# GuyTevet/motion-diffusion-model

Measured on NVIDIA H100. Metric: motions/sec, higher is better.
Workload: dtype fp16 operands / fp32 accumulate (in/out projections hi-lo split)

## Files before the change

motion-diffusion-model_b200/csrc/attention_tc.cuh:

```cuda
#pragma once
#include <cuda_fp16.h>

#include "epilogues.cuh"
#include "ptx.cuh"

namespace b200 {

constexpr int ATC_THREADS = 256;
constexpr int ATC_QROWS = 128;
constexpr int ATC_DH = 128;
constexpr int ATC_MAX_KEYS = 256;

struct AttnTcSmem {
  static __host__ __device__ int total(int keys) { return 1024 + 4 * keys * 128; }
};

template <bool WIDE>
__global__ void __launch_bounds__(ATC_THREADS, 2)
attention_tc_kernel(const __grid_constant__ CUtensorMap map_kv, const __half* __restrict__ qkv, __half* __restrict__ out,
                    const int* __restrict__ kvlen, int S, int d, int keys, float scale_log2) {
  extern __shared__ uint8_t smem_raw[];
  __shared__ uint64_t bar_k, bar_v;
  const int atom = keys * 128;
  uint8_t* sK = reinterpret_cast<uint8_t*>((reinterpret_cast<uintptr_t>(smem_raw) + 1023) & ~uintptr_t(1023));
  uint8_t* sV = sK + 2 * atom;
  const int warp = threadIdx.x >> 5, lane = threadIdx.x & 31;
  const int h = blockIdx.x, smp = blockIdx.y, tile = blockIdx.z;
  const int ld = 3 * d;
  const __half* base = qkv + static_cast<size_t>(smp) * S * ld;

  pdl_launch_dependents();
  if (threadIdx.x == 0) {
    tma_prefetch_desc(&map_kv);
    mbar_init(&bar_k, 1);
    mbar_init(&bar_v, 1);
    fence_barrier_init();
  }
  __syncthreads();
  pdl_wait();
  if (threadIdx.x == 0) {
    mbar_expect_tx(&bar_k, 2 * atom);
    for (int a = 0; a < 2; ++a) tma_load_3d(sK + a * atom, &map_kv, &bar_k, d + h * ATC_DH + 64 * a, 0, smp);
    mbar_expect_tx(&bar_v, 2 * atom);
    for (int a = 0; a < 2; ++a) tma_load_3d(sV + a * atom, &map_kv, &bar_v, 2 * d + h * ATC_DH + 64 * a, 0, smp);
  }

  const int q0 = tile * ATC_QROWS + warp * 16;
  if (q0 >= S) return;
  const int g = lane >> 2, t = lane & 3;
  const int ra = q0 + g, rb = q0 + g + 8;
  const bool va = ra < S, vb = rb < S;
  uint32_t qa[8][4];
  {
    const uint32_t* pa = reinterpret_cast<const uint32_t*>(base + static_cast<size_t>(va ? ra : 0) * ld + h * ATC_DH);
    const uint32_t* pb = reinterpret_cast<const uint32_t*>(base + static_cast<size_t>(vb ? rb : 0) * ld + h * ATC_DH);
#pragma unroll
    for (int ks = 0; ks < 8; ++ks) {
      qa[ks][0] = va ? pa[8 * ks + t] : 0u;
      qa[ks][1] = vb ? pb[8 * ks + t] : 0u;
      qa[ks][2] = va ? pa[8 * ks + 4 + t] : 0u;
      qa[ks][3] = vb ? pb[8 * ks + 4 + t] : 0u;
    }
  }
  const int kvl = min(kvlen[smp], S);
  const int nblk = max(1, (kvl + 15) >> 4);
  const uint32_t r7 = lane & 7;
  const uint32_t k_row = smem_u32(sK) + ((lane & 7) + 8 * (lane >> 4)) * 128, k_hi = (lane >> 3) & 1;
  const uint32_t v_row = smem_u32(sV) + ((lane & 7) + 8 * ((lane >> 3) & 1)) * 128, v_hi = lane >> 4;
  auto swz = [&](uint32_t row_addr, uint32_t chunk) {
    return row_addr + (chunk >> 3) * atom + (((chunk & 7) ^ r7) << 4);
  };
  auto scores = [&](int kk, float (&s)[2][4]) {
#pragma unroll
    for (int n = 0; n < 2; ++n)
#pragma unroll
      for (int i = 0; i < 4; ++i) s[n][i] = 0.f;
#pragma unroll
    for (int ks = 0; ks < 8; ++ks) {
      uint32_t b[4];
      ldmatrix_x4(b, swz(k_row + 16 * kk * 128, 2 * ks + k_hi));
      mma_16816(s[0], qa[ks], b[0], b[1]);
      mma_16816(s[1], qa[ks], b[2], b[3]);
    }
  };
  mbar_wait(&bar_k, 0);
  float mxa = -INFINITY, mxb = -INFINITY;
#pragma unroll 1
  for (int kk = 0; kk < nblk; ++kk) {
    float s[2][4];
    scores(kk, s);
#pragma unroll
    for (int n = 0; n < 2; ++n)
#pragma unroll
      for (int i = 0; i < 2; ++i) {
        const int key = 16 * kk + 8 * n + 2 * t + i;
        if (key < kvl) {
          mxa = fmaxf(mxa, s[n][i]);
          mxb = fmaxf(mxb, s[n][2 + i]);
        }
      }
  }
#pragma unroll
  for (int o = 1; o < 4; o <<= 1) {
    mxa = fmaxf(mxa, __shfl_xor_sync(0xffffffffu, mxa, o));
    mxb = fmaxf(mxb, __shfl_xor_sync(0xffffffffu, mxb, o));
  }
  const float offa = (mxa == -INFINITY) ? 0.f : mxa * scale_log2;
  const float offb = (mxb == -INFINITY) ? 0.f : mxb * scale_log2;
  auto ex2 = [](float x) {
    float y;
    asm("ex2.approx.ftz.f32 %0, %1;" : "=f"(y) : "f"(x));
    return y;
  };
  float o[16][4];
#pragma unroll
  for (int j = 0; j < 16; ++j)
#pragma unroll
    for (int i = 0; i < 4; ++i) o[j][i] = 0.f;
  float suma = 0.f, sumb = 0.f;
  mbar_wait(&bar_v, 0);
#pragma unroll 1
  for (int kk = 0; kk < nblk; ++kk) {
    float s[2][4];
    scores(kk, s);
    uint32_t pa[4];
#pragma unroll
    for (int n = 0; n < 2; ++n) {
      const int key = 16 * kk + 8 * n + 2 * t;
      const float p0 = key < kvl ? ex2(fmaf(s[n][0], scale_log2, -offa)) : 0.f;
      const float p1 = key + 1 < kvl ? ex2(fmaf(s[n][1], scale_log2, -offa)) : 0.f;
      const float p2 = key < kvl ? ex2(fmaf(s[n][2], scale_log2, -offb)) : 0.f;
      const float p3 = key + 1 < kvl ? ex2(fmaf(s[n][3], scale_log2, -offb)) : 0.f;
      suma += p0 + p1;
      sumb += p2 + p3;
      pa[2 * n] = pack_half2(p0, p1);
      pa[2 * n + 1] = pack_half2(p2, p3);
    }
#pragma unroll
    for (int nd = 0; nd < 8; ++nd) {
      uint32_t b[4];
      ldmatrix_x4_trans(b, swz(v_row + 16 * kk * 128, 2 * nd + v_hi));
      mma_16816(o[2 * nd], pa, b[0], b[1]);
      mma_16816(o[2 * nd + 1], pa, b[2], b[3]);
    }
  }
#pragma unroll
  for (int off = 1; off < 4; off <<= 1) {
    suma += __shfl_xor_sync(0xffffffffu, suma, off);
    sumb += __shfl_xor_sync(0xffffffffu, sumb, off);
  }
  const float inva = suma > 0.f ? 1.f / suma : 0.f;
  const float invb = sumb > 0.f ? 1.f / sumb : 0.f;
  const int ldo = (WIDE ? 2 : 1) * d;
  __half* oa = out + (static_cast<size_t>(smp) * S + (va ? ra : 0)) * ldo + h * ATC_DH + 2 * t;
  __half* ob = out + (static_cast<size_t>(smp) * S + (vb ? rb : 0)) * ldo + h * ATC_DH + 2 * t;
#pragma unroll
  for (int j = 0; j < 16; ++j) {
    const float x0 = o[j][0] * inva, x1 = o[j][1] * inva, x2 = o[j][2] * invb, x3 = o[j][3] * invb;
    const __half2 ha = __floats2half2_rn(x0, x1), hb = __floats2half2_rn(x2, x3);
    if (va) *reinterpret_cast<__half2*>(oa + 8 * j) = ha;
    if (vb) *reinterpret_cast<__half2*>(ob + 8 * j) = hb;
    if (WIDE) {
      const float2 fa = __half22float2(ha), fb = __half22float2(hb);
      if (va) *reinterpret_cast<__half2*>(oa + d + 8 * j) = __floats2half2_rn(x0 - fa.x, x1 - fa.y);
      if (vb) *reinterpret_cast<__half2*>(ob + d + 8 * j) = __floats2half2_rn(x2 - fb.x, x3 - fb.y);
    }
  }
}

}
```

motion-diffusion-model_b200/csrc/engine.cu:

```cuda
#include <cuda.h>
#include <cuda_fp16.h>
#include <cuda_runtime.h>

#include <cmath>
#include <cstdarg>
#include <cstdio>
#include <cstring>
#include <map>
#include <string>
#include <vector>

#include "../../include/b200mdm.h"
#include "attention_tc.cuh"
#include "epilogues.cuh"
#include "gemm.cuh"
#include "gemm_ln.cuh"
#include "postprocess.cuh"
#include "kernels.cuh"

using namespace b200;

static thread_local char g_err[512] = "";
static int fail(int code, const char* fmt, ...) {
  va_list ap;
// ... 166 lines not shown
  if (zero) CUDA_TRY(cudaMemset(*p, 0, n * sizeof(T)));
  return B200MDM_OK;
}
template <class T>
static void dfree(T*& p) {
  if (p) cudaFree(p);
  p = nullptr;
}

template <int BN, class Epi, bool RES = false>
static int set_gemm_attr() {
  CUDA_TRY(cudaFuncSetAttribute(gemm_f16_wgmma<BN, Epi, RES>, cudaFuncAttributeMaxDynamicSharedMemorySize,
                                GemmSmem<BN, Epi, RES>::TOTAL));
  return B200MDM_OK;
}
static int init_kernel_attrs() {
  static unsigned long long done_mask = 0;
  int dev = 0;
  CUDA_TRY(cudaGetDevice(&dev));
  if (dev < 64 && ((done_mask >> dev) & 1ull)) return B200MDM_OK;
  TRY((set_gemm_attr<128, EpiBiasF16<false>>()));
  TRY((set_gemm_attr<128, EpiBiasF16<true>>()));
  TRY((set_gemm_attr<256, EpiBiasF16<false>>()));
  TRY((set_gemm_attr<256, EpiBiasF16<true>>()));
  TRY((set_gemm_attr<64, EpiBiasF16<false>, true>()));
  TRY((set_gemm_attr<64, EpiBiasF16<true>, true>()));
  TRY((set_gemm_attr<128, EpiBiasF16Wide<true>>()));
  TRY((set_gemm_attr<128, EpiBiasF16Global>()));
  CUDA_TRY(cudaFuncSetAttribute(gemm_resid_ln_cluster, cudaFuncAttributeMaxDynamicSharedMemorySize, GemmLnSmem::TOTAL));
  TRY((set_gemm_attr<128, EpiEmbed>()));
  TRY((set_gemm_attr<96, EpiOutStep>()));
  CUDA_TRY(cudaFuncSetAttribute(attention_tc_kernel<false>, cudaFuncAttributeMaxDynamicSharedMemorySize,
                                AttnTcSmem::total(ATC_MAX_KEYS)));
  CUDA_TRY(cudaFuncSetAttribute(attention_tc_kernel<true>, cudaFuncAttributeMaxDynamicSharedMemorySize,
                                AttnTcSmem::total(ATC_MAX_KEYS)));
  if (dev < 64) done_mask |= 1ull << dev;
  return B200MDM_OK;
}

static bool g_pdl_now = false;
static bool pdl_enabled() {
  static int v = -1;
  if (v < 0) {
    const char* e = getenv("B200MDM_PDL");
    v = (e && e[0] == '0') ? 0 : 1;
  }
  return v == 1;
}
struct PdlScope {
  PdlScope() { g_pdl_now = pdl_enabled(); }
// ... 44 lines not shown
                            const float* bias, cudaStream_t s, int num_sms) {
  typename EpiBiasF16<GELU>::Params p{bias};
  return launch_gemm<128, EpiBiasF16<GELU>>(a, b, c, M, N, K, p, s, num_sms);
}

static int launch_gemm_resid_ln(const CUtensorMap& a, const CUtensorMap& w256, const CUtensorMap& hres, int M, int K,
                                const float* bias, const float* gamma, const float* beta, cudaStream_t s, int num_sms) {
  const int tiles = (M + GEMM_BLOCK_M - 1) / GEMM_BLOCK_M;
  const int max_clusters = num_sms / 2;
  const int clusters = tiles < max_clusters ? tiles : max_clusters;
  GemmLnParams lp{bias, gamma, beta, 1e-5f};
  CUDA_TRY(launch_k(gemm_resid_ln_cluster, dim3(2 * clusters), dim3(GLN_THREADS), GemmLnSmem::TOTAL, s, a, w256, hres, M, K, lp));
  return B200MDM_OK;
}

static int launch_attention_tc(const CUtensorMap& map_kv, const __half* qkv, __half* out, const int* kvlen, int n_samples,
                               int S, int d, int H, cudaStream_t s, bool wide = false) {
  if (d != H * ATC_DH) return fail(B200MDM_ENOTIMPL, "attention: head_dim must be 128");
  if (S > ATC_MAX_KEYS) return fail(B200MDM_ENOTIMPL, "attention: at most %d tokens per sample", ATC_MAX_KEYS);
  const int keys = (S + 15) & ~15;
  const float scale_log2 = 1.4426950408889634f / sqrtf(static_cast<float>(ATC_DH));
  const dim3 grid(H, n_samples, (S + ATC_QROWS - 1) / ATC_QROWS);
  CUDA_TRY(launch_k(wide ? attention_tc_kernel<true> : attention_tc_kernel<false>, grid, dim3(ATC_THREADS), AttnTcSmem::total(keys),
                    s, map_kv, qkv, out, kvlen, S, d, keys, scale_log2));
  return B200MDM_OK;
}
#ifdef B200_TRACE
static int debug_skip_mask() {
  static int v = -1;
  if (v < 0) {
    const char* e = getenv("B200MDM_DEBUG_SKIP");
    v = e ? atoi(e) : 0;
  }
  return v;
}
#define B200_SKIP(bit) (debug_skip_mask() & (bit))
#else
#define B200_SKIP(bit) (0)
#endif
// ... 299 lines not shown
  if (e->dec) {
    TRY(dalloc(&e->qc16, M * d));
    TRY(make_map_t(&e->m_qc_st, e->qc16, 2, M, d, d, 32));
    e->Mt = 0;
    e->prefix_set = false;
  }
  e->B = B; e->T = T; e->S = S; e->halves = halves; e->Bp = Bp;
  e->M = static_cast<int>(M); e->MB = static_cast<int>(MB);
  attach_l2_window(e);
  TRY(make_map(&e->m_xin, e->xin16, MB, 3 * e->Kp_in, 3 * e->Kp_in, GEMM_BLOCK_M));
  TRY(make_map(&e->m_h16, e->hres, M, kw * d, 2 * d, GEMM_BLOCK_M));
  TRY(make_map(&e->m_att, e->att16, M, kw * d, kw * d, GEMM_BLOCK_M));
  TRY(make_map(&e->m_ffn, e->ffn16, M, kw * e->ff, kw * e->ff, GEMM_BLOCK_M));
  TRY(make_map(&e->m_g16, e->g16, static_cast<size_t>(B) * T, 3 * d, 3 * d, GEMM_BLOCK_M));
  TRY(make_map_t(&e->m_qkv_st, e->qkv16, 2, M, 3 * d, 3 * d, 32));
  TRY(make_map_3d(&e->m_qkv_kv, e->qkv16, Bp, S, 3 * d, 3 * d, (S + 15) & ~15));
  TRY(make_map_t(&e->m_ffn_st, e->ffn16, 2, M, kw * e->ff, kw * e->ff, 32));
  TRY(make_map_res(&e->m_res_c, e->hres, MB, d));
  TRY(make_map_res(&e->m_res_u, e->hres + (halves == 2 ? MB * d * 2 : 0), MB, d));
  TRY(make_hres_map(&e->m_hres, e->hres, M));
  TRY(dalloc(&e->pe_bias, static_cast<size_t>(S) * d));
  pe_bias_kernel<<<S, 128, 0, s>>>(e->pe_bias, e->pe, e->b_in, S, d);
  CUDA_TRY(cudaGetLastError());
  TRY(dalloc(&e->eps_buf, static_cast<size_t>(B) * e->JF * T));
  return B200MDM_OK;
}

static void attach_l2_window(b200mdm_engine* e, cudaStream_t stream) {
  cudaDeviceProp prop;
  int dev = 0;
  if (cudaGetDevice(&dev) == cudaSuccess && cudaGetDeviceProperties(&prop, dev) == cudaSuccess && prop.persistingL2CacheMaxSize > 0) {
// ... 632 lines not shown
  p.noise_batch_stride = (flags & B200MDM_FLAG_CONST_NOISE) ? 0 : static_cast<long long>(JF) * T;
  p.B = B; p.S = T; p.T = T; p.J = JF; p.mode = mode;
  p.s_off = 0;
  p.clip_denoised = (flags & B200MDM_FLAG_CLIP_DENOISED) ? 1 : 0;
  return launch_gemm<96, EpiOutStep>(m_g16, m_wout, m_g16, B * T, N_out_pad, 3 * d, p, s, sms);
}

extern "C" int b200mdm_test_attention(const void* qkv16_dev, void* out16_dev, const int32_t* kvlen_dev,
                                      int32_t n_samples, int32_t S, int32_t d, int32_t impl, void* stream) {
  if (!qkv16_dev || !out16_dev || !kvlen_dev || n_samples <= 0 || S <= 0) return fail(B200MDM_EINVAL, "bad argument");
  TRY(init_kernel_attrs());
  cudaStream_t s = static_cast<cudaStream_t>(stream);
  if (impl != 0 && impl != 1) return fail(B200MDM_EINVAL, "impl must be 0 (fp16 output) or 1 ([hi | lo] output)");
  if (S > ATC_MAX_KEYS) return fail(B200MDM_EINVAL, "attention handles at most %d tokens", ATC_MAX_KEYS);
  CUtensorMap mkv;
  TRY(make_map_3d(&mkv, qkv16_dev, n_samples, S, 3 * d, 3 * d, (S + 15) & ~15));
  return launch_attention_tc(mkv, static_cast<const __half*>(qkv16_dev), static_cast<__half*>(out16_dev), kvlen_dev, n_samples,
                             S, d, d / ATC_DH, s, impl == 1);
}

extern "C" int b200mdm_test_cross_attention(const void* q16_dev, const void* kv16_dev, const unsigned char* mask_dev,
                                            void* out16_dev, int32_t n_samples, int32_t S, int32_t n_tokens, int32_t ld_kv,
                                            void* stream) {
  const int d = 512;
  if (!q16_dev || !kv16_dev || !mask_dev || !out16_dev || n_samples <= 0 || S <= 0 || n_tokens <= 0 || n_tokens > 64 ||
      ld_kv < 2 * d || ld_kv % 8)
    return fail(B200MDM_EINVAL, "bad argument");
  cudaStream_t s = static_cast<cudaStream_t>(stream);
  const float sl2 = 1.4426950408889634f / sqrtf(128.0f);
  const dim3 cg(d / 128, n_samples), cb(128);
  const __half* q = static_cast<const __half*>(q16_dev);
// ... 12 lines not shown
      ld < 512 || ld % 8)
    return fail(B200MDM_EINVAL, "bad argument");
  TRY(init_kernel_attrs());
  int dev = 0, sms = 132;
  CUDA_TRY(cudaGetDevice(&dev));
  CUDA_TRY(cudaDeviceGetAttribute(&sms, cudaDevAttrMultiProcessorCount, dev));
  cudaStream_t s = static_cast<cudaStream_t>(stream);
  const int M = n_samples * S;
  __half* qkv = nullptr;
  CUDA_TRY(cudaMallocAsync(reinterpret_cast<void**>(&qkv), static_cast<size_t>(M) * 1536 * sizeof(__half), s));
  CUtensorMap ma, mb, mc, mkv;
  int r = make_map(&ma, h16_dev, M, 512, ld, GEMM_BLOCK_M);
  if (r == B200MDM_OK) r = make_map(&mb, wqkv16_dev, 1536, 512, 512, 128);
  if (r == B200MDM_OK) r = make_map_t(&mc, qkv, 2, M, 1536, 1536, 32);
  if (r == B200MDM_OK) r = launch_gemm_bias<false>(ma, mb, mc, M, 1536, 512, bqkv_dev, s, sms);
  if (r == B200MDM_OK) r = make_map_3d(&mkv, qkv, n_samples, S, 1536, 1536, (S + 15) & ~15);
  if (r == B200MDM_OK)
    r = launch_attention_tc(mkv, qkv, static_cast<__half*>(out16_dev), kvlen_dev, n_samples, S, 512, 4, s);
  CUDA_TRY(cudaFreeAsync(qkv, s));
  return r;
}

extern "C" int b200mdm_test_gemm_resid_ln(const void* a16_dev, const void* w16_dev, const float* bias_dev,
                                          const float* gamma_dev, const float* beta_dev, void* hres16_dev, int32_t M,
                                          int32_t K, void* stream) {
  if (!a16_dev || !w16_dev || !bias_dev || !gamma_dev || !beta_dev || !hres16_dev || M <= 0 || K <= 0 || K % 8)
    return fail(B200MDM_EINVAL, "bad argument");
  TRY(init_kernel_attrs());
  int dev = 0, sms = 132;
  CUDA_TRY(cudaGetDevice(&dev));
  CUDA_TRY(cudaDeviceGetAttribute(&sms, cudaDevAttrMultiProcessorCount, dev));
// ... 25 lines not shown
```

motion-diffusion-model_b200/csrc/ptx.cuh:

```cuda
#pragma once
#include <cuda.h>
#include <cuda_fp16.h>
#include <cuda_runtime.h>
#include <stdint.h>

namespace b200 {

__device__ __forceinline__ uint32_t smem_u32(const void* p) {
  return static_cast<uint32_t>(__cvta_generic_to_shared(p));
}

__device__ __forceinline__ bool elect_one() {
  uint32_t pred = 0;
  asm volatile(
      "{\n\t.reg .pred P;\n\t"
      "elect.sync _|P, 0xffffffff;\n\t"
      "selp.u32 %0, 1, 0, P;\n\t}\n"
      : "=r"(pred));
  return pred != 0;
}

__device__ __forceinline__ void mbar_init(uint64_t* bar, uint32_t count) {
  asm volatile("mbarrier.init.shared::cta.b64 [%0], %1;" ::"r"(smem_u32(bar)), "r"(count) : "memory");
}
// ... 106 lines not shown
}
__device__ __forceinline__ void st_async_f32x2(uint32_t remote_addr, float a, float b, uint32_t remote_bar) {
  asm volatile("st.async.shared::cluster.mbarrier::complete_tx::bytes.v2.f32 [%0], {%1, %2}, [%3];"
               ::"r"(remote_addr), "f"(a), "f"(b), "r"(remote_bar)
               : "memory");
}

__device__ __forceinline__ uint64_t wgmma_desc_k_sw128(uint32_t smem_addr) {
  uint64_t d = 0;
  d |= static_cast<uint64_t>((smem_addr & 0x3FFFF) >> 4);
  d |= static_cast<uint64_t>(1) << 16;
  d |= static_cast<uint64_t>(1024 >> 4) << 32;
  d |= static_cast<uint64_t>(1) << 62;
  return d;
}
__device__ __forceinline__ void wgmma_fence() { asm volatile("wgmma.fence.sync.aligned;" ::: "memory"); }
__device__ __forceinline__ void wgmma_commit() { asm volatile("wgmma.commit_group.sync.aligned;" ::: "memory"); }
template <int N>
__device__ __forceinline__ void wgmma_wait() {
  asm volatile("wgmma.wait_group.sync.aligned %0;" ::"n"(N) : "memory");
}
template <int NR>
__device__ __forceinline__ void wgmma_fence_acc(float (&d)[NR]) {
#pragma unroll
  for (int i = 0; i < NR; ++i) asm volatile("" : "+f"(d[i])::"memory");
}

template <int N> struct Wgmma;
#include "wgmma_ops.inc"

__device__ __forceinline__ void mma_16816(float (&c)[4], const uint32_t (&a)[4], uint32_t b0, uint32_t b1) {
  asm volatile("mma.sync.aligned.m16n8k16.row.col.f32.f16.f16.f32 {%0,%1,%2,%3}, {%4,%5,%6,%7}, {%8,%9}, {%0,%1,%2,%3};\n"
               : "+f"(c[0]), "+f"(c[1]), "+f"(c[2]), "+f"(c[3])
               : "r"(a[0]), "r"(a[1]), "r"(a[2]), "r"(a[3]), "r"(b0), "r"(b1));
}
__device__ __forceinline__ void ldmatrix_x4(uint32_t (&r)[4], uint32_t smem_addr) {
  asm volatile("ldmatrix.sync.aligned.m8n8.x4.shared.b16 {%0,%1,%2,%3}, [%4];"
               : "=r"(r[0]), "=r"(r[1]), "=r"(r[2]), "=r"(r[3]) : "r"(smem_addr));
}
__device__ __forceinline__ void ldmatrix_x4_trans(uint32_t (&r)[4], uint32_t smem_addr) {
  asm volatile("ldmatrix.sync.aligned.m8n8.x4.trans.shared.b16 {%0,%1,%2,%3}, [%4];"
               : "=r"(r[0]), "=r"(r[1]), "=r"(r[2]), "=r"(r[3]) : "r"(smem_addr));
}
// ... 3 lines not shown
```

motion-diffusion-model_b200/csrc/wgmma_ops.inc:

```
template <> struct Wgmma<64> {
  static constexpr int NREG = 32;
  static __device__ __forceinline__ void mma(float (&d)[32], uint64_t da, uint64_t db, uint32_t accumulate) {
    asm volatile(
        "{\n\t.reg .pred p;\n\tsetp.ne.b32 p, %34, 0;\n\t"
        "wgmma.mma_async.sync.aligned.m64n64k16.f32.f16.f16 {%0, %1, %2, %3, %4, %5, %6, %7, %8, %9, %10, %11, %12, %13, %14, %15, %16, %17, %18, %19, %20, %21, %22, %23, %24, %25, %26, %27, %28, %29, %30, %31}, %32, %33, p, 1, 1, 0, 0;\n\t}\n"
        : "+f"(d[0]), "+f"(d[1]), "+f"(d[2]), "+f"(d[3]), "+f"(d[4]), "+f"(d[5]), "+f"(d[6]), "+f"(d[7]), "+f"(d[8]), "+f"(d[9]), "+f"(d[10]), "+f"(d[11]), "+f"(d[12]), "+f"(d[13]), "+f"(d[14]), "+f"(d[15]), "+f"(d[16]), "+f"(d[17]), "+f"(d[18]), "+f"(d[19]), "+f"(d[20]), "+f"(d[21]), "+f"(d[22]), "+f"(d[23]), "+f"(d[24]), "+f"(d[25]), "+f"(d[26]), "+f"(d[27]), "+f"(d[28]), "+f"(d[29]), "+f"(d[30]), "+f"(d[31])
        : "l"(da), "l"(db), "r"(accumulate));
  }
};
template <> struct Wgmma<96> {
  static constexpr int NREG = 48;
  static __device__ __forceinline__ void mma(float (&d)[48], uint64_t da, uint64_t db, uint32_t accumulate) {
    asm volatile(
        "{\n\t.reg .pred p;\n\tsetp.ne.b32 p, %50, 0;\n\t"
        "wgmma.mma_async.sync.aligned.m64n96k16.f32.f16.f16 {%0, %1, %2, %3, %4, %5, %6, %7, %8, %9, %10, %11, %12, %13, %14, %15, %16, %17, %18, %19, %20, %21, %22, %23, %24, %25, %26, %27, %28, %29, %30, %31, %32, %33, %34, %35, %36, %37, %38, %39, %40, %41, %42, %43, %44, %45, %46, %47}, %48, %49, p, 1, 1, 0, 0;\n\t}\n"
        : "+f"(d[0]), "+f"(d[1]), "+f"(d[2]), "+f"(d[3]), "+f"(d[4]), "+f"(d[5]), "+f"(d[6]), "+f"(d[7]), "+f"(d[8]), "+f"(d[9]), "+f"(d[10]), "+f"(d[11]), "+f"(d[12]), "+f"(d[13]), "+f"(d[14]), "+f"(d[15]), "+f"(d[16]), "+f"(d[17]), "+f"(d[18]), "+f"(d[19]), "+f"(d[20]), "+f"(d[21]), "+f"(d[22]), "+f"(d[23]), "+f"(d[24]), "+f"(d[25]), "+f"(d[26]), "+f"(d[27]), "+f"(d[28]), "+f"(d[29]), "+f"(d[30]), "+f"(d[31]), "+f"(d[32]), "+f"(d[33]), "+f"(d[34]), "+f"(d[35]), "+f"(d[36]), "+f"(d[37]), "+f"(d[38]), "+f"(d[39]), "+f"(d[40]), "+f"(d[41]), "+f"(d[42]), "+f"(d[43]), "+f"(d[44]), "+f"(d[45]), "+f"(d[46]), "+f"(d[47])
        : "l"(da), "l"(db), "r"(accumulate));
  }
};
template <> struct Wgmma<128> {
  static constexpr int NREG = 64;
  static __device__ __forceinline__ void mma(float (&d)[64], uint64_t da, uint64_t db, uint32_t accumulate) {
    asm volatile(
        "{\n\t.reg .pred p;\n\tsetp.ne.b32 p, %66, 0;\n\t"
        "wgmma.mma_async.sync.aligned.m64n128k16.f32.f16.f16 {%0, %1, %2, %3, %4, %5, %6, %7, %8, %9, %10, %11, %12, %13, %14, %15, %16, %17, %18, %19, %20, %21, %22, %23, %24, %25, %26, %27, %28, %29, %30, %31, %32, %33, %34, %35, %36, %37, %38, %39, %40, %41, %42, %43, %44, %45, %46, %47, %48, %49, %50, %51, %52, %53, %54, %55, %56, %57, %58, %59, %60, %61, %62, %63}, %64, %65, p, 1, 1, 0, 0;\n\t}\n"
        : "+f"(d[0]), "+f"(d[1]), "+f"(d[2]), "+f"(d[3]), "+f"(d[4]), "+f"(d[5]), "+f"(d[6]), "+f"(d[7]), "+f"(d[8]), "+f"(d[9]), "+f"(d[10]), "+f"(d[11]), "+f"(d[12]), "+f"(d[13]), "+f"(d[14]), "+f"(d[15]), "+f"(d[16]), "+f"(d[17]), "+f"(d[18]), "+f"(d[19]), "+f"(d[20]), "+f"(d[21]), "+f"(d[22]), "+f"(d[23]), "+f"(d[24]), "+f"(d[25]), "+f"(d[26]), "+f"(d[27]), "+f"(d[28]), "+f"(d[29]), "+f"(d[30]), "+f"(d[31]), "+f"(d[32]), "+f"(d[33]), "+f"(d[34]), "+f"(d[35]), "+f"(d[36]), "+f"(d[37]), "+f"(d[38]), "+f"(d[39]), "+f"(d[40]), "+f"(d[41]), "+f"(d[42]), "+f"(d[43]), "+f"(d[44]), "+f"(d[45]), "+f"(d[46]), "+f"(d[47]), "+f"(d[48]), "+f"(d[49]), "+f"(d[50]), "+f"(d[51]), "+f"(d[52]), "+f"(d[53]), "+f"(d[54]), "+f"(d[55]), "+f"(d[56]), "+f"(d[57]), "+f"(d[58]), "+f"(d[59]), "+f"(d[60]), "+f"(d[61]), "+f"(d[62]), "+f"(d[63])
        : "l"(da), "l"(db), "r"(accumulate));
  }
};
template <> struct Wgmma<256> {
  static constexpr int NREG = 128;
  static __device__ __forceinline__ void mma(float (&d)[128], uint64_t da, uint64_t db, uint32_t accumulate) {
    asm volatile(
        "{\n\t.reg .pred p;\n\tsetp.ne.b32 p, %130, 0;\n\t"
        "wgmma.mma_async.sync.aligned.m64n256k16.f32.f16.f16 {%0, %1, %2, %3, %4, %5, %6, %7, %8, %9, %10, %11, %12, %13, %14, %15, %16, %17, %18, %19, %20, %21, %22, %23, %24, %25, %26, %27, %28, %29, %30, %31, %32, %33, %34, %35, %36, %37, %38, %39, %40, %41, %42, %43, %44, %45, %46, %47, %48, %49, %50, %51, %52, %53, %54, %55, %56, %57, %58, %59, %60, %61, %62, %63, %64, %65, %66, %67, %68, %69, %70, %71, %72, %73, %74, %75, %76, %77, %78, %79, %80, %81, %82, %83, %84, %85, %86, %87, %88, %89, %90, %91, %92, %93, %94, %95, %96, %97, %98, %99, %100, %101, %102, %103, %104, %105, %106, %107, %108, %109, %110, %111, %112, %113, %114, %115, %116, %117, %118, %119, %120, %121, %122, %123, %124, %125, %126, %127}, %128, %129, p, 1, 1, 0, 0;\n\t}\n"
        : "+f"(d[0]), "+f"(d[1]), "+f"(d[2]), "+f"(d[3]), "+f"(d[4]), "+f"(d[5]), "+f"(d[6]), "+f"(d[7]), "+f"(d[8]), "+f"(d[9]), "+f"(d[10]), "+f"(d[11]), "+f"(d[12]), "+f"(d[13]), "+f"(d[14]), "+f"(d[15]), "+f"(d[16]), "+f"(d[17]), "+f"(d[18]), "+f"(d[19]), "+f"(d[20]), "+f"(d[21]), "+f"(d[22]), "+f"(d[23]), "+f"(d[24]), "+f"(d[25]), "+f"(d[26]), "+f"(d[27]), "+f"(d[28]), "+f"(d[29]), "+f"(d[30]), "+f"(d[31]), "+f"(d[32]), "+f"(d[33]), "+f"(d[34]), "+f"(d[35]), "+f"(d[36]), "+f"(d[37]), "+f"(d[38]), "+f"(d[39]), "+f"(d[40]), "+f"(d[41]), "+f"(d[42]), "+f"(d[43]), "+f"(d[44]), "+f"(d[45]), "+f"(d[46]), "+f"(d[47]), "+f"(d[48]), "+f"(d[49]), "+f"(d[50]), "+f"(d[51]), "+f"(d[52]), "+f"(d[53]), "+f"(d[54]), "+f"(d[55]), "+f"(d[56]), "+f"(d[57]), "+f"(d[58]), "+f"(d[59]), "+f"(d[60]), "+f"(d[61]), "+f"(d[62]), "+f"(d[63]), "+f"(d[64]), "+f"(d[65]), "+f"(d[66]), "+f"(d[67]), "+f"(d[68]), "+f"(d[69]), "+f"(d[70]), "+f"(d[71]), "+f"(d[72]), "+f"(d[73]), "+f"(d[74]), "+f"(d[75]), "+f"(d[76]), "+f"(d[77]), "+f"(d[78]), "+f"(d[79]), "+f"(d[80]), "+f"(d[81]), "+f"(d[82]), "+f"(d[83]), "+f"(d[84]), "+f"(d[85]), "+f"(d[86]), "+f"(d[87]), "+f"(d[88]), "+f"(d[89]), "+f"(d[90]), "+f"(d[91]), "+f"(d[92]), "+f"(d[93]), "+f"(d[94]), "+f"(d[95]), "+f"(d[96]), "+f"(d[97]), "+f"(d[98]), "+f"(d[99]), "+f"(d[100]), "+f"(d[101]), "+f"(d[102]), "+f"(d[103]), "+f"(d[104]), "+f"(d[105]), "+f"(d[106]), "+f"(d[107]), "+f"(d[108]), "+f"(d[109]), "+f"(d[110]), "+f"(d[111]), "+f"(d[112]), "+f"(d[113]), "+f"(d[114]), "+f"(d[115]), "+f"(d[116]), "+f"(d[117]), "+f"(d[118]), "+f"(d[119]), "+f"(d[120]), "+f"(d[121]), "+f"(d[122]), "+f"(d[123]), "+f"(d[124]), "+f"(d[125]), "+f"(d[126]), "+f"(d[127])
        : "l"(da), "l"(db), "r"(accumulate));
  }
};
```

Measured before the change: 335.6.

## Rewrite attention kernel with register-A wgmma and persistent multi-tile CTAs

```diff
diff --git a/motion-diffusion-model_b200/csrc/attention_tc.cuh b/motion-diffusion-model_b200/csrc/attention_tc.cuh
--- a/motion-diffusion-model_b200/csrc/attention_tc.cuh
+++ b/motion-diffusion-model_b200/csrc/attention_tc.cuh
@@ -6,26 +6,31 @@
 
 namespace b200 {
 
-constexpr int ATC_THREADS = 256;
-constexpr int ATC_QROWS = 128;
+constexpr int ATC_THREADS = 128;
+constexpr int ATC_QROWS = 64;
+constexpr int ATC_TILES_PER_CTA = 4;
 constexpr int ATC_DH = 128;
 constexpr int ATC_MAX_KEYS = 256;
+
+__host__ __device__ constexpr int atc_keys(int S) { return S <= 64 ? 64 : S <= 208 ? 208 : 256; }
 
 struct AttnTcSmem {
   static __host__ __device__ int total(int keys) { return 1024 + 4 * keys * 128; }
 };
 
-template <bool WIDE>
+template <int KEYS, bool WIDE>
 __global__ void __launch_bounds__(ATC_THREADS, 2)
 attention_tc_kernel(const __grid_constant__ CUtensorMap map_kv, const __half* __restrict__ qkv, __half* __restrict__ out,
-                    const int* __restrict__ kvlen, int S, int d, int keys, float scale_log2) {
+                    const int* __restrict__ kvlen, int S, int d, float scale_log2) {
+  constexpr int ATOM = KEYS * 128;
+  constexpr int NS = KEYS / 2;
+  constexpr int NB = KEYS / 16;
   extern __shared__ uint8_t smem_raw[];
   __shared__ uint64_t bar_k, bar_v;
-  const int atom = keys * 128;
   uint8_t* sK = reinterpret_cast<uint8_t*>((reinterpret_cast<uintptr_t>(smem_raw) + 1023) & ~uintptr_t(1023));
-  uint8_t* sV = sK + 2 * atom;
+  uint8_t* sV = sK + 2 * ATOM;
   const int warp = threadIdx.x >> 5, lane = threadIdx.x & 31;
-  const int h = blockIdx.x, smp = blockIdx.y, tile = blockIdx.z;
+  const int h = blockIdx.x, smp = blockIdx.y;
   const int ld = 3 * d;
   const __half* base = qkv + static_cast<size_t>(smp) * S * ld;
 
@@ -39,19 +44,24 @@
   __syncthreads();
   pdl_wait();
   if (threadIdx.x == 0) {
-    mbar_expect_tx(&bar_k, 2 * atom);
-    for (int a = 0; a < 2; ++a) tma_load_3d(sK + a * atom, &map_kv, &bar_k, d + h * ATC_DH + 64 * a, 0, smp);
-    mbar_expect_tx(&bar_v, 2 * atom);
-    for (int a = 0; a < 2; ++a) tma_load_3d(sV + a * atom, &map_kv, &bar_v, 2 * d + h * ATC_DH + 64 * a, 0, smp);
+    mbar_expect_tx(&bar_k, 2 * ATOM);
+    for (int a = 0; a < 2; ++a) tma_load_3d(sK + a * ATOM, &map_kv, &bar_k, d + h * ATC_DH + 64 * a, 0, smp);
+    mbar_expect_tx(&bar_v, 2 * ATOM);
+    for (int a = 0; a < 2; ++a) tma_load_3d(sV + a * ATOM, &map_kv, &bar_v, 2 * d + h * ATC_DH + 64 * a, 0, smp);
   }
 
-  const int q0 = tile * ATC_QROWS + warp * 16;
-  if (q0 >= S) return;
+  const int kvl = min(kvlen[smp], S);
+  const int nblk = max(1, (kvl + 15) >> 4);
   const int g = lane >> 2, t = lane & 3;
-  const int ra = q0 + g, rb = q0 + g + 8;
-  const bool va = ra < S, vb = rb < S;
+  const uint64_t desc_k = wgmma_desc_k_sw128(smem_u32(sK));
+  const uint64_t desc_v = wgmma_desc_mn_sw128(smem_u32(sV), ATOM);
+  const int ntiles = (S + ATC_QROWS - 1) / ATC_QROWS;
+  const int ldo = (WIDE ? 2 : 1) * d;
+
   uint32_t qa[8][4];
-  {
+  auto load_q = [&](int tile) {
+    const int ra = tile * ATC_QROWS + warp * 16 + g, rb = ra + 8;
+    const bool va = ra < S, vb = rb < S;
     const uint32_t* pa = reinterpret_cast<const uint32_t*>(base + static_cast<size_t>(va ? ra : 0) * ld + h * ATC_DH);
     const uint32_t* pb = reinterpret_cast<const uint32_t*>(base + static_cast<size_t>(vb ? rb : 0) * ld + h * ATC_DH);
 #pragma unroll
@@ -61,109 +71,87 @@
       qa[ks][2] = va ? pa[8 * ks + 4 + t] : 0u;
       qa[ks][3] = vb ? pb[8 * ks + 4 + t] : 0u;
     }
-  }
-  const int kvl = min(kvlen[smp], S);
-  const int nblk = max(1, (kvl + 15) >> 4);
-  const uint32_t r7 = lane & 7;
-  const uint32_t k_row = smem_u32(sK) + ((lane & 7) + 8 * (lane >> 4)) * 128, k_hi = (lane >> 3) & 1;
-  const uint32_t v_row = smem_u32(sV) + ((lane & 7) + 8 * ((lane >> 3) & 1)) * 128, v_hi = lane >> 4;
-  auto swz = [&](uint32_t row_addr, uint32_t chunk) {
-    return row_addr + (chunk >> 3) * atom + (((chunk & 7) ^ r7) << 4);
   };
-  auto scores = [&](int kk, float (&s)[2][4]) {
+  if (static_cast<int>(blockIdx.z) < ntiles) load_q(blockIdx.z);
+#pragma unroll 1
+  for (int tile = blockIdx.z; tile < ntiles; tile += gridDim.z) {
+    const int ra = tile * ATC_QROWS + warp * 16 + g, rb = ra + 8;
+    const bool va = ra < S, vb = rb < S;
+    float s[NS];
+    mbar_wait(&bar_k, 0);
+    wgmma_fence();
 #pragma unroll
-    for (int n = 0; n < 2; ++n)
+    for (int ks = 0; ks < 8; ++ks)
+      WgmmaRA<KEYS, 0>::mma(s, qa[ks], desc_k + (((ks >> 2) * ATOM + (ks & 3) * 32) >> 4), ks != 0);
+    wgmma_commit();
+    wgmma_wait<0>();
+    wgmma_fence_acc(s);
+    float mxa = -INFINITY, mxb = -INFINITY;
 #pragma unroll
-      for (int i = 0; i < 4; ++i) s[n][i] = 0.f;
-#pragma unroll
-    for (int ks = 0; ks < 8; ++ks) {
-      uint32_t b[4];
-      ldmatrix_x4(b, swz(k_row + 16 * kk * 128, 2 * ks + k_hi));
-      mma_16816(s[0], qa[ks], b[0], b[1]);
-      mma_16816(s[1], qa[ks], b[2], b[3]);
-    }
-  };
-  mbar_wait(&bar_k, 0);
-  float mxa = -INFINITY, mxb = -INFINITY;
-#pragma unroll 1
-  for (int kk = 0; kk < nblk; ++kk) {
-    float s[2][4];
-    scores(kk, s);
-#pragma unroll
-    for (int n = 0; n < 2; ++n)
+    for (int j = 0; j < NS / 4; ++j)
 #pragma unroll
       for (int i = 0; i < 2; ++i) {
-        const int key = 16 * kk + 8 * n + 2 * t + i;
-        if (key < kvl) {
-          mxa = fmaxf(mxa, s[n][i]);
-          mxb = fmaxf(mxb, s[n][2 + i]);
+        if (8 * j + 2 * t + i < kvl) {
+          mxa = fmaxf(mxa, s[4 * j + i]);
+          mxb = fmaxf(mxb, s[4 * j + 2 + i]);
         }
       }
-  }
 #pragma unroll
-  for (int o = 1; o < 4; o <<= 1) {
-    mxa = fmaxf(mxa, __shfl_xor_sync(0xffffffffu, mxa, o));
-    mxb = fmaxf(mxb, __shfl_xor_sync(0xffffffffu, mxb, o));
-  }
-  const float offa = (mxa == -INFINITY) ? 0.f : mxa * scale_log2;
-  const float offb = (mxb == -INFINITY) ? 0.f : mxb * scale_log2;
-  auto ex2 = [](float x) {
-    float y;
-    asm("ex2.approx.ftz.f32 %0, %1;" : "=f"(y) : "f"(x));
-    return y;
-  };
-  float o[16][4];
+    for (int o = 1; o < 4; o <<= 1) {
+      mxa = fmaxf(mxa, __shfl_xor_sync(0xffffffffu, mxa, o));
+      mxb = fmaxf(mxb, __shfl_xor_sync(0xffffffffu, mxb, o));
+    }
+    const float offa = (mxa == -INFINITY) ? 0.f : mxa * scale_log2;
+    const float offb = (mxb == -INFINITY) ? 0.f : mxb * scale_log2;
+    auto ex2 = [](float x) {
+      float y;
+      asm("ex2.approx.ftz.f32 %0, %1;" : "=f"(y) : "f"(x));
+      return y;
+    };
+    uint32_t p[NB][4];
+    float suma = 0.f, sumb = 0.f;
 #pragma unroll
-  for (int j = 0; j < 16; ++j)
-#pragma unroll
-    for (int i = 0; i < 4; ++i) o[j][i] = 0.f;
-  float suma = 0.f, sumb = 0.f;
-  mbar_wait(&bar_v, 0);
-#pragma unroll 1
-  for (int kk = 0; kk < nblk; ++kk) {
-    float s[2][4];
-    scores(kk, s);
-    uint32_t pa[4];
-#pragma unroll
-    for (int n = 0; n < 2; ++n) {
-      const int key = 16 * kk + 8 * n + 2 * t;
-      const float p0 = key < kvl ? ex2(fmaf(s[n][0], scale_log2, -offa)) : 0.f;
-      const float p1 = key + 1 < kvl ? ex2(fmaf(s[n][1], scale_log2, -offa)) : 0.f;
-      const float p2 = key < kvl ? ex2(fmaf(s[n][2], scale_log2, -offb)) : 0.f;
-      const float p3 = key + 1 < kvl ? ex2(fmaf(s[n][3], scale_log2, -offb)) : 0.f;
+    for (int j = 0; j < NS / 4; ++j) {
+      const int key = 8 * j + 2 * t;
+      const float p0 = key < kvl ? ex2(fmaf(s[4 * j], scale_log2, -offa)) : 0.f;
+      const float p1 = key + 1 < kvl ? ex2(fmaf(s[4 * j + 1], scale_log2, -offa)) : 0.f;
+      const float p2 = key < kvl ? ex2(fmaf(s[4 * j + 2], scale_log2, -offb)) : 0.f;
+      const float p3 = key + 1 < kvl ? ex2(fmaf(s[4 * j + 3], scale_log2, -offb)) : 0.f;
       suma += p0 + p1;
       sumb += p2 + p3;
-      pa[2 * n] = pack_half2(p0, p1);
-      pa[2 * n + 1] = pack_half2(p2, p3);
+      p[j >> 1][2 * (j & 1)] = pack_half2(p0, p1);
+      p[j >> 1][2 * (j & 1) + 1] = pack_half2(p2, p3);
     }
 #pragma unroll
-    for (int nd = 0; nd < 8; ++nd) {
-      uint32_t b[4];
-      ldmatrix_x4_trans(b, swz(v_row + 16 * kk * 128, 2 * nd + v_hi));
-      mma_16816(o[2 * nd], pa, b[0], b[1]);
-      mma_16816(o[2 * nd + 1], pa, b[2], b[3]);
+    for (int off = 1; off < 4; off <<= 1) {
+      suma += __shfl_xor_sync(0xffffffffu, suma, off);
+      sumb += __shfl_xor_sync(0xffffffffu, sumb, off);
     }
-  }
+    const float inva = suma > 0.f ? 1.f / suma : 0.f;
+    const float invb = sumb > 0.f ? 1.f / sumb : 0.f;
+    float o[64];
+    mbar_wait(&bar_v, 0);
+    wgmma_fence();
 #pragma unroll
-  for (int off = 1; off < 4; off <<= 1) {
-    suma += __shfl_xor_sync(0xffffffffu, suma, off);
-    sumb += __shfl_xor_sync(0xffffffffu, sumb, off);
-  }
-  const float inva = suma > 0.f ? 1.f / suma : 0.f;
-  const float invb = sumb > 0.f ? 1.f / sumb : 0.f;
-  const int ldo = (WIDE ? 2 : 1) * d;
-  __half* oa = out + (static_cast<size_t>(smp) * S + (va ? ra : 0)) * ldo + h * ATC_DH + 2 * t;
-  __half* ob = out + (static_cast<size_t>(smp) * S + (vb ? rb : 0)) * ldo + h * ATC_DH + 2 * t;
+    for (int kk = 0; kk < NB; ++kk)
+      if (kk < nblk) WgmmaRA<128, 1>::mma(o, p[kk], desc_v + ((kk * 16 * 128) >> 4), kk != 0);
+    wgmma_commit();
+    if (tile + static_cast<int>(gridDim.z) < ntiles) load_q(tile + gridDim.z);
+    wgmma_wait<0>();
+    wgmma_fence_acc(o);
+    __half* oa = out + (static_cast<size_t>(smp) * S + (va ? ra : 0)) * ldo + h * ATC_DH + 2 * t;
+    __half* ob = out + (static_cast<size_t>(smp) * S + (vb ? rb : 0)) * ldo + h * ATC_DH + 2 * t;
 #pragma unroll
-  for (int j = 0; j < 16; ++j) {
-    const float x0 = o[j][0] * inva, x1 = o[j][1] * inva, x2 = o[j][2] * invb, x3 = o[j][3] * invb;
-    const __half2 ha = __floats2half2_rn(x0, x1), hb = __floats2half2_rn(x2, x3);
-    if (va) *reinterpret_cast<__half2*>(oa + 8 * j) = ha;
-    if (vb) *reinterpret_cast<__half2*>(ob + 8 * j) = hb;
-    if (WIDE) {
-      const float2 fa = __half22float2(ha), fb = __half22float2(hb);
-      if (va) *reinterpret_cast<__half2*>(oa + d + 8 * j) = __floats2half2_rn(x0 - fa.x, x1 - fa.y);
-      if (vb) *reinterpret_cast<__half2*>(ob + d + 8 * j) = __floats2half2_rn(x2 - fb.x, x3 - fb.y);
+    for (int j = 0; j < 16; ++j) {
+      const float x0 = o[4 * j] * inva, x1 = o[4 * j + 1] * inva, x2 = o[4 * j + 2] * invb, x3 = o[4 * j + 3] * invb;
+      const __half2 ha = __floats2half2_rn(x0, x1), hb = __floats2half2_rn(x2, x3);
+      if (va) *reinterpret_cast<__half2*>(oa + 8 * j) = ha;
+      if (vb) *reinterpret_cast<__half2*>(ob + 8 * j) = hb;
+      if (WIDE) {
+        const float2 fa = __half22float2(ha), fb = __half22float2(hb);
+        if (va) *reinterpret_cast<__half2*>(oa + d + 8 * j) = __floats2half2_rn(x0 - fa.x, x1 - fa.y);
+        if (vb) *reinterpret_cast<__half2*>(ob + d + 8 * j) = __floats2half2_rn(x2 - fb.x, x3 - fb.y);
+      }
     }
   }
 }
diff --git a/motion-diffusion-model_b200/csrc/engine.cu b/motion-diffusion-model_b200/csrc/engine.cu
--- a/motion-diffusion-model_b200/csrc/engine.cu
+++ b/motion-diffusion-model_b200/csrc/engine.cu
@@ -204,6 +204,14 @@
                                 GemmSmem<BN, Epi, RES>::TOTAL));
   return B200MDM_OK;
 }
+template <int KEYS>
+static int set_attention_attr() {
+  CUDA_TRY(cudaFuncSetAttribute(attention_tc_kernel<KEYS, false>, cudaFuncAttributeMaxDynamicSharedMemorySize,
+                                AttnTcSmem::total(KEYS)));
+  CUDA_TRY(cudaFuncSetAttribute(attention_tc_kernel<KEYS, true>, cudaFuncAttributeMaxDynamicSharedMemorySize,
+                                AttnTcSmem::total(KEYS)));
+  return B200MDM_OK;
+}
 static int init_kernel_attrs() {
   static unsigned long long done_mask = 0;
   int dev = 0;
@@ -220,10 +228,9 @@
   CUDA_TRY(cudaFuncSetAttribute(gemm_resid_ln_cluster, cudaFuncAttributeMaxDynamicSharedMemorySize, GemmLnSmem::TOTAL));
   TRY((set_gemm_attr<128, EpiEmbed>()));
   TRY((set_gemm_attr<96, EpiOutStep>()));
-  CUDA_TRY(cudaFuncSetAttribute(attention_tc_kernel<false>, cudaFuncAttributeMaxDynamicSharedMemorySize,
-                                AttnTcSmem::total(ATC_MAX_KEYS)));
-  CUDA_TRY(cudaFuncSetAttribute(attention_tc_kernel<true>, cudaFuncAttributeMaxDynamicSharedMemorySize,
-                                AttnTcSmem::total(ATC_MAX_KEYS)));
+  TRY((set_attention_attr<64>()));
+  TRY((set_attention_attr<208>()));
+  TRY((set_attention_attr<256>()));
   if (dev < 64) done_mask |= 1ull << dev;
   return B200MDM_OK;
 }
@@ -298,15 +305,26 @@
   return B200MDM_OK;
 }
 
+static int make_attention_kv_map(CUtensorMap* m, const void* qkv, int n_samples, int S, int ld) {
+  return make_map_3d(m, qkv, n_samples, S, ld, ld, atc_keys(S));
+}
+template <int KEYS>
+static cudaError_t launch_attention_keys(const CUtensorMap& map_kv, const __half* qkv, __half* out, const int* kvlen,
+                                         dim3 grid, int S, int d, float scale_log2, cudaStream_t s, bool wide) {
+  return launch_k(wide ? attention_tc_kernel<KEYS, true> : attention_tc_kernel<KEYS, false>, grid, dim3(ATC_THREADS),
+                  AttnTcSmem::total(KEYS), s, map_kv, qkv, out, kvlen, S, d, scale_log2);
+}
 static int launch_attention_tc(const CUtensorMap& map_kv, const __half* qkv, __half* out, const int* kvlen, int n_samples,
                                int S, int d, int H, cudaStream_t s, bool wide = false) {
   if (d != H * ATC_DH) return fail(B200MDM_ENOTIMPL, "attention: head_dim must be 128");
   if (S > ATC_MAX_KEYS) return fail(B200MDM_ENOTIMPL, "attention: at most %d tokens per sample", ATC_MAX_KEYS);
-  const int keys = (S + 15) & ~15;
   const float scale_log2 = 1.4426950408889634f / sqrtf(static_cast<float>(ATC_DH));
-  const dim3 grid(H, n_samples, (S + ATC_QROWS - 1) / ATC_QROWS);
-  CUDA_TRY(launch_k(wide ? attention_tc_kernel<true> : attention_tc_kernel<false>, grid, dim3(ATC_THREADS), AttnTcSmem::total(keys),
-                    s, map_kv, qkv, out, kvlen, S, d, keys, scale_log2));
+  const int tiles = (S + ATC_QROWS - 1) / ATC_QROWS;
+  const dim3 grid(H, n_samples, (tiles + ATC_TILES_PER_CTA - 1) / ATC_TILES_PER_CTA);
+  const int keys = atc_keys(S);
+  if (keys == 64) CUDA_TRY(launch_attention_keys<64>(map_kv, qkv, out, kvlen, grid, S, d, scale_log2, s, wide));
+  else if (keys == 208) CUDA_TRY(launch_attention_keys<208>(map_kv, qkv, out, kvlen, grid, S, d, scale_log2, s, wide));
+  else CUDA_TRY(launch_attention_keys<256>(map_kv, qkv, out, kvlen, grid, S, d, scale_log2, s, wide));
   return B200MDM_OK;
 }
 #ifdef B200_TRACE
@@ -636,7 +654,7 @@
   TRY(make_map(&e->m_ffn, e->ffn16, M, kw * e->ff, kw * e->ff, GEMM_BLOCK_M));
   TRY(make_map(&e->m_g16, e->g16, static_cast<size_t>(B) * T, 3 * d, 3 * d, GEMM_BLOCK_M));
   TRY(make_map_t(&e->m_qkv_st, e->qkv16, 2, M, 3 * d, 3 * d, 32));
-  TRY(make_map_3d(&e->m_qkv_kv, e->qkv16, Bp, S, 3 * d, 3 * d, (S + 15) & ~15));
+  TRY(make_attention_kv_map(&e->m_qkv_kv, e->qkv16, Bp, S, 3 * d));
   TRY(make_map_t(&e->m_ffn_st, e->ffn16, 2, M, kw * e->ff, kw * e->ff, 32));
   TRY(make_map_res(&e->m_res_c, e->hres, MB, d));
   TRY(make_map_res(&e->m_res_u, e->hres + (halves == 2 ? MB * d * 2 : 0), MB, d));
@@ -1299,7 +1317,7 @@
   if (impl != 0 && impl != 1) return fail(B200MDM_EINVAL, "impl must be 0 (fp16 output) or 1 ([hi | lo] output)");
   if (S > ATC_MAX_KEYS) return fail(B200MDM_EINVAL, "attention handles at most %d tokens", ATC_MAX_KEYS);
   CUtensorMap mkv;
-  TRY(make_map_3d(&mkv, qkv16_dev, n_samples, S, 3 * d, 3 * d, (S + 15) & ~15));
+  TRY(make_attention_kv_map(&mkv, qkv16_dev, n_samples, S, 3 * d));
   return launch_attention_tc(mkv, static_cast<const __half*>(qkv16_dev), static_cast<__half*>(out16_dev), kvlen_dev, n_samples,
                              S, d, d / ATC_DH, s, impl == 1);
 }
@@ -1342,7 +1360,7 @@
   if (r == B200MDM_OK) r = make_map(&mb, wqkv16_dev, 1536, 512, 512, 128);
   if (r == B200MDM_OK) r = make_map_t(&mc, qkv, 2, M, 1536, 1536, 32);
   if (r == B200MDM_OK) r = launch_gemm_bias<false>(ma, mb, mc, M, 1536, 512, bqkv_dev, s, sms);
-  if (r == B200MDM_OK) r = make_map_3d(&mkv, qkv, n_samples, S, 1536, 1536, (S + 15) & ~15);
+  if (r == B200MDM_OK) r = make_attention_kv_map(&mkv, qkv, n_samples, S, 1536);
   if (r == B200MDM_OK)
     r = launch_attention_tc(mkv, qkv, static_cast<__half*>(out16_dev), kvlen_dev, n_samples, S, 512, 4, s);
   CUDA_TRY(cudaFreeAsync(qkv, s));
diff --git a/motion-diffusion-model_b200/csrc/ptx.cuh b/motion-diffusion-model_b200/csrc/ptx.cuh
--- a/motion-diffusion-model_b200/csrc/ptx.cuh
+++ b/motion-diffusion-model_b200/csrc/ptx.cuh
@@ -144,6 +144,14 @@
   d |= static_cast<uint64_t>(1) << 62;
   return d;
 }
+__device__ __forceinline__ uint64_t wgmma_desc_mn_sw128(uint32_t smem_addr, uint32_t mn_atom_bytes) {
+  uint64_t d = 0;
+  d |= static_cast<uint64_t>((smem_addr & 0x3FFFF) >> 4);
+  d |= static_cast<uint64_t>((mn_atom_bytes >> 4) & 0x3FFF) << 16;
+  d |= static_cast<uint64_t>(1024 >> 4) << 32;
+  d |= static_cast<uint64_t>(1) << 62;
+  return d;
+}
 __device__ __forceinline__ void wgmma_fence() { asm volatile("wgmma.fence.sync.aligned;" ::: "memory"); }
 __device__ __forceinline__ void wgmma_commit() { asm volatile("wgmma.commit_group.sync.aligned;" ::: "memory"); }
 template <int N>
@@ -157,6 +165,7 @@
 }
 
 template <int N> struct Wgmma;
+template <int N, int TRANS_B> struct WgmmaRA;
 #include "wgmma_ops.inc"
 
 __device__ __forceinline__ void mma_16816(float (&c)[4], const uint32_t (&a)[4], uint32_t b0, uint32_t b1) {
diff --git a/motion-diffusion-model_b200/csrc/wgmma_ops.inc b/motion-diffusion-model_b200/csrc/wgmma_ops.inc
--- a/motion-diffusion-model_b200/csrc/wgmma_ops.inc
+++ b/motion-diffusion-model_b200/csrc/wgmma_ops.inc
@@ -38,3 +38,43 @@
         : "l"(da), "l"(db), "r"(accumulate));
   }
 };
+template <> struct WgmmaRA<64, 0> {
+  static constexpr int NREG = 32;
+  static __device__ __forceinline__ void mma(float (&d)[32], const uint32_t (&a)[4], uint64_t db, uint32_t accumulate) {
+    asm volatile(
+        "{\n\t.reg .pred p;\n\tsetp.ne.b32 p, %37, 0;\n\t"
+        "wgmma.mma_async.sync.aligned.m64n64k16.f32.f16.f16 {%0, %1, %2, %3, %4, %5, %6, %7, %8, %9, %10, %11, %12, %13, %14, %15, %16, %17, %18, %19, %20, %21, %22, %23, %24, %25, %26, %27, %28, %29, %30, %31}, {%32, %33, %34, %35}, %36, p, 1, 1, 0;\n\t}\n"
+        : "+f"(d[0]), "+f"(d[1]), "+f"(d[2]), "+f"(d[3]), "+f"(d[4]), "+f"(d[5]), "+f"(d[6]), "+f"(d[7]), "+f"(d[8]), "+f"(d[9]), "+f"(d[10]), "+f"(d[11]), "+f"(d[12]), "+f"(d[13]), "+f"(d[14]), "+f"(d[15]), "+f"(d[16]), "+f"(d[17]), "+f"(d[18]), "+f"(d[19]), "+f"(d[20]), "+f"(d[21]), "+f"(d[22]), "+f"(d[23]), "+f"(d[24]), "+f"(d[25]), "+f"(d[26]), "+f"(d[27]), "+f"(d[28]), "+f"(d[29]), "+f"(d[30]), "+f"(d[31])
+        : "r"(a[0]), "r"(a[1]), "r"(a[2]), "r"(a[3]), "l"(db), "r"(accumulate));
+  }
+};
+template <> struct WgmmaRA<208, 0> {
+  static constexpr int NREG = 104;
+  static __device__ __forceinline__ void mma(float (&d)[104], const uint32_t (&a)[4], uint64_t db, uint32_t accumulate) {
+    asm volatile(
+        "{\n\t.reg .pred p;\n\tsetp.ne.b32 p, %109, 0;\n\t"
+        "wgmma.mma_async.sync.aligned.m64n208k16.f32.f16.f16 {%0, %1, %2, %3, %4, %5, %6, %7, %8, %9, %10, %11, %12, %13, %14, %15, %16, %17, %18, %19, %20, %21, %22, %23, %24, %25, %26, %27, %28, %29, %30, %31, %32, %33, %34, %35, %36, %37, %38, %39, %40, %41, %42, %43, %44, %45, %46, %47, %48, %49, %50, %51, %52, %53, %54, %55, %56, %57, %58, %59, %60, %61, %62, %63, %64, %65, %66, %67, %68, %69, %70, %71, %72, %73, %74, %75, %76, %77, %78, %79, %80, %81, %82, %83, %84, %85, %86, %87, %88, %89, %90, %91, %92, %93, %94, %95, %96, %97, %98, %99, %100, %101, %102, %103}, {%104, %105, %106, %107}, %108, p, 1, 1, 0;\n\t}\n"
+        : "+f"(d[0]), "+f"(d[1]), "+f"(d[2]), "+f"(d[3]), "+f"(d[4]), "+f"(d[5]), "+f"(d[6]), "+f"(d[7]), "+f"(d[8]), "+f"(d[9]), "+f"(d[10]), "+f"(d[11]), "+f"(d[12]), "+f"(d[13]), "+f"(d[14]), "+f"(d[15]), "+f"(d[16]), "+f"(d[17]), "+f"(d[18]), "+f"(d[19]), "+f"(d[20]), "+f"(d[21]), "+f"(d[22]), "+f"(d[23]), "+f"(d[24]), "+f"(d[25]), "+f"(d[26]), "+f"(d[27]), "+f"(d[28]), "+f"(d[29]), "+f"(d[30]), "+f"(d[31]), "+f"(d[32]), "+f"(d[33]), "+f"(d[34]), "+f"(d[35]), "+f"(d[36]), "+f"(d[37]), "+f"(d[38]), "+f"(d[39]), "+f"(d[40]), "+f"(d[41]), "+f"(d[42]), "+f"(d[43]), "+f"(d[44]), "+f"(d[45]), "+f"(d[46]), "+f"(d[47]), "+f"(d[48]), "+f"(d[49]), "+f"(d[50]), "+f"(d[51]), "+f"(d[52]), "+f"(d[53]), "+f"(d[54]), "+f"(d[55]), "+f"(d[56]), "+f"(d[57]), "+f"(d[58]), "+f"(d[59]), "+f"(d[60]), "+f"(d[61]), "+f"(d[62]), "+f"(d[63]), "+f"(d[64]), "+f"(d[65]), "+f"(d[66]), "+f"(d[67]), "+f"(d[68]), "+f"(d[69]), "+f"(d[70]), "+f"(d[71]), "+f"(d[72]), "+f"(d[73]), "+f"(d[74]), "+f"(d[75]), "+f"(d[76]), "+f"(d[77]), "+f"(d[78]), "+f"(d[79]), "+f"(d[80]), "+f"(d[81]), "+f"(d[82]), "+f"(d[83]), "+f"(d[84]), "+f"(d[85]), "+f"(d[86]), "+f"(d[87]), "+f"(d[88]), "+f"(d[89]), "+f"(d[90]), "+f"(d[91]), "+f"(d[92]), "+f"(d[93]), "+f"(d[94]), "+f"(d[95]), "+f"(d[96]), "+f"(d[97]), "+f"(d[98]), "+f"(d[99]), "+f"(d[100]), "+f"(d[101]), "+f"(d[102]), "+f"(d[103])
+        : "r"(a[0]), "r"(a[1]), "r"(a[2]), "r"(a[3]), "l"(db), "r"(accumulate));
+  }
+};
+template <> struct WgmmaRA<256, 0> {
+  static constexpr int NREG = 128;
+  static __device__ __forceinline__ void mma(float (&d)[128], const uint32_t (&a)[4], uint64_t db, uint32_t accumulate) {
+    asm volatile(
+        "{\n\t.reg .pred p;\n\tsetp.ne.b32 p, %133, 0;\n\t"
+        "wgmma.mma_async.sync.aligned.m64n256k16.f32.f16.f16 {%0, %1, %2, %3, %4, %5, %6, %7, %8, %9, %10, %11, %12, %13, %14, %15, %16, %17, %18, %19, %20, %21, %22, %23, %24, %25, %26, %27, %28, %29, %30, %31, %32, %33, %34, %35, %36, %37, %38, %39, %40, %41, %42, %43, %44, %45, %46, %47, %48, %49, %50, %51, %52, %53, %54, %55, %56, %57, %58, %59, %60, %61, %62, %63, %64, %65, %66, %67, %68, %69, %70, %71, %72, %73, %74, %75, %76, %77, %78, %79, %80, %81, %82, %83, %84, %85, %86, %87, %88, %89, %90, %91, %92, %93, %94, %95, %96, %97, %98, %99, %100, %101, %102, %103, %104, %105, %106, %107, %108, %109, %110, %111, %112, %113, %114, %115, %116, %117, %118, %119, %120, %121, %122, %123, %124, %125, %126, %127}, {%128, %129, %130, %131}, %132, p, 1, 1, 0;\n\t}\n"
+        : "+f"(d[0]), "+f"(d[1]), "+f"(d[2]), "+f"(d[3]), "+f"(d[4]), "+f"(d[5]), "+f"(d[6]), "+f"(d[7]), "+f"(d[8]), "+f"(d[9]), "+f"(d[10]), "+f"(d[11]), "+f"(d[12]), "+f"(d[13]), "+f"(d[14]), "+f"(d[15]), "+f"(d[16]), "+f"(d[17]), "+f"(d[18]), "+f"(d[19]), "+f"(d[20]), "+f"(d[21]), "+f"(d[22]), "+f"(d[23]), "+f"(d[24]), "+f"(d[25]), "+f"(d[26]), "+f"(d[27]), "+f"(d[28]), "+f"(d[29]), "+f"(d[30]), "+f"(d[31]), "+f"(d[32]), "+f"(d[33]), "+f"(d[34]), "+f"(d[35]), "+f"(d[36]), "+f"(d[37]), "+f"(d[38]), "+f"(d[39]), "+f"(d[40]), "+f"(d[41]), "+f"(d[42]), "+f"(d[43]), "+f"(d[44]), "+f"(d[45]), "+f"(d[46]), "+f"(d[47]), "+f"(d[48]), "+f"(d[49]), "+f"(d[50]), "+f"(d[51]), "+f"(d[52]), "+f"(d[53]), "+f"(d[54]), "+f"(d[55]), "+f"(d[56]), "+f"(d[57]), "+f"(d[58]), "+f"(d[59]), "+f"(d[60]), "+f"(d[61]), "+f"(d[62]), "+f"(d[63]), "+f"(d[64]), "+f"(d[65]), "+f"(d[66]), "+f"(d[67]), "+f"(d[68]), "+f"(d[69]), "+f"(d[70]), "+f"(d[71]), "+f"(d[72]), "+f"(d[73]), "+f"(d[74]), "+f"(d[75]), "+f"(d[76]), "+f"(d[77]), "+f"(d[78]), "+f"(d[79]), "+f"(d[80]), "+f"(d[81]), "+f"(d[82]), "+f"(d[83]), "+f"(d[84]), "+f"(d[85]), "+f"(d[86]), "+f"(d[87]), "+f"(d[88]), "+f"(d[89]), "+f"(d[90]), "+f"(d[91]), "+f"(d[92]), "+f"(d[93]), "+f"(d[94]), "+f"(d[95]), "+f"(d[96]), "+f"(d[97]), "+f"(d[98]), "+f"(d[99]), "+f"(d[100]), "+f"(d[101]), "+f"(d[102]), "+f"(d[103]), "+f"(d[104]), "+f"(d[105]), "+f"(d[106]), "+f"(d[107]), "+f"(d[108]), "+f"(d[109]), "+f"(d[110]), "+f"(d[111]), "+f"(d[112]), "+f"(d[113]), "+f"(d[114]), "+f"(d[115]), "+f"(d[116]), "+f"(d[117]), "+f"(d[118]), "+f"(d[119]), "+f"(d[120]), "+f"(d[121]), "+f"(d[122]), "+f"(d[123]), "+f"(d[124]), "+f"(d[125]), "+f"(d[126]), "+f"(d[127])
+        : "r"(a[0]), "r"(a[1]), "r"(a[2]), "r"(a[3]), "l"(db), "r"(accumulate));
+  }
+};
+template <> struct WgmmaRA<128, 1> {
+  static constexpr int NREG = 64;
+  static __device__ __forceinline__ void mma(float (&d)[64], const uint32_t (&a)[4], uint64_t db, uint32_t accumulate) {
+    asm volatile(
+        "{\n\t.reg .pred p;\n\tsetp.ne.b32 p, %69, 0;\n\t"
+        "wgmma.mma_async.sync.aligned.m64n128k16.f32.f16.f16 {%0, %1, %2, %3, %4, %5, %6, %7, %8, %9, %10, %11, %12, %13, %14, %15, %16, %17, %18, %19, %20, %21, %22, %23, %24, %25, %26, %27, %28, %29, %30, %31, %32, %33, %34, %35, %36, %37, %38, %39, %40, %41, %42, %43, %44, %45, %46, %47, %48, %49, %50, %51, %52, %53, %54, %55, %56, %57, %58, %59, %60, %61, %62, %63}, {%64, %65, %66, %67}, %68, p, 1, 1, 1;\n\t}\n"
+        : "+f"(d[0]), "+f"(d[1]), "+f"(d[2]), "+f"(d[3]), "+f"(d[4]), "+f"(d[5]), "+f"(d[6]), "+f"(d[7]), "+f"(d[8]), "+f"(d[9]), "+f"(d[10]), "+f"(d[11]), "+f"(d[12]), "+f"(d[13]), "+f"(d[14]), "+f"(d[15]), "+f"(d[16]), "+f"(d[17]), "+f"(d[18]), "+f"(d[19]), "+f"(d[20]), "+f"(d[21]), "+f"(d[22]), "+f"(d[23]), "+f"(d[24]), "+f"(d[25]), "+f"(d[26]), "+f"(d[27]), "+f"(d[28]), "+f"(d[29]), "+f"(d[30]), "+f"(d[31]), "+f"(d[32]), "+f"(d[33]), "+f"(d[34]), "+f"(d[35]), "+f"(d[36]), "+f"(d[37]), "+f"(d[38]), "+f"(d[39]), "+f"(d[40]), "+f"(d[41]), "+f"(d[42]), "+f"(d[43]), "+f"(d[44]), "+f"(d[45]), "+f"(d[46]), "+f"(d[47]), "+f"(d[48]), "+f"(d[49]), "+f"(d[50]), "+f"(d[51]), "+f"(d[52]), "+f"(d[53]), "+f"(d[54]), "+f"(d[55]), "+f"(d[56]), "+f"(d[57]), "+f"(d[58]), "+f"(d[59]), "+f"(d[60]), "+f"(d[61]), "+f"(d[62]), "+f"(d[63])
+        : "r"(a[0]), "r"(a[1]), "r"(a[2]), "r"(a[3]), "l"(db), "r"(accumulate));
+  }
+};
```

After: 354.9, median of 6. 1.06x the previous value.
